# apache/datafusion-comet

Measured on NVIDIA H100. Metric: rows/sec on TPC-H Q1 filter+agg, higher is better.
Workload: dtype i128

## Files before the change

### datafusion-comet_b200/csrc/agg.cpp

```cpp
#include "exec_internal.h"
#include "../../include/comet_b200.h"

#include "aot_kernels.h"
#include "ranges.h"

#include <algorithm>
#include <mutex>

namespace cb200 {

static std::mutex g_profile_mu;
static std::map<std::string, std::vector<int>> g_range_profile;

void reset_range_profiles() {
    std::lock_guard<std::mutex> lk(g_profile_mu);
    g_range_profile.clear();
}

namespace {

enum class Strategy { Undecided, Dense, Table, Stream };
enum Level { SAFE = 0, TYPE = 1, TIGHT = 2 };
constexpr int DENSE_MAX_GROUPS = 64;

// ... 3 lines not shown

using ValueMasks = uint64_t[CB_MAX_COLS * 2];

uint64_t identity_word(int kind) { return kind == W_MIN ? 0x7fffffffffffffffull : kind == W_MAX ? 0x8000000000000000ull : 0; }

std::vector<int> decode_gid(int g, const std::vector<int>& cards) {
    std::vector<int> code(cards.size());
    for (int k = (int)cards.size() - 1; k >= 0; k--) { code[(size_t)k] = g % cards[(size_t)k]; g /= cards[(size_t)k]; }
    return code;
}

int grid_for(const ExecContext* ctx, int n_tiles) { return std::max(1, std::min(ctx->num_sms, n_tiles)); }

struct Kernel {
    PipelineSpec spec;
    GeneratedKernel g;
    std::shared_ptr<CompiledModule> mod;
};

void launch_named(ExecContext* ctx, const Kernel& k, const char* name, dim3 grid, dim3 block, void** args) {
    cuda_check(cudaLaunchKernel((const void*)k.mod->kernel(name), grid, block, args, 0, ctx->stream), name);
    ctx->kernel_launches++;
}

struct DenseState {
    std::vector<int> cards;
    std::vector<bool> has_null;
    DeviceBufP totals, spill, partials;
    int groups = 0;

    void regroup(ExecContext* ctx, int n_words, const std::vector<int>& word_kinds, const std::vector<int>& new_cards) {
        int new_groups = 1;
// ... 7 lines not shown
            for (int k = (int)cards.size() - 1; k >= 0; k--) {
                int cd = code[(size_t)k];
                if (has_null[(size_t)k] && cd == cards[(size_t)k] - 1) cd = new_cards[(size_t)k] - 1;
                ng += cd * mul;
                mul *= new_cards[(size_t)k];
            }
            memcpy(&newt[(size_t)ng * n_words * 2], &oldt[(size_t)g * n_words * 2], (size_t)n_words * 16);
        }
        totals = host_to_device(newt.data(), newt.size() * 8, ctx, "regroup H2D");
        groups = new_groups;
    }

    void finalize(ExecContext* ctx, const Kernel& last, cb::FinParams fp, bool ungrouped, const std::vector<DType>& schema,
                  const std::vector<DictionaryP>& key_dicts, Batch& out) const {
        TraceSpan ts("agg.finalize");
        const GeneratedKernel& g = last.g;
        const int ng = groups;
        fp.totals = (cb::u64*)totals->ptr;
        fp.n_groups = ng;
        std::vector<size_t> off_v, off_n;
        size_t total_bytes = 0;
        auto take = [&](size_t n) { size_t o = total_bytes; total_bytes += (n + 15) / 16 * 16; return o; };
        for (size_t i = 0; i < g.out_cols.size(); i++) { off_v.push_back(take((size_t)ng * g.out_bytes[i])); off_n.push_back(take((size_t)ng)); }
        size_t off_present = take((size_t)ng);
        auto dbuf = std::make_shared<DeviceBuf>(total_bytes);
        for (size_t i = 0; i < g.out_cols.size(); i++) {
            fp.out[i] = (cb::u8*)dbuf->ptr + off_v[i];
            fp.outv[i] = (cb::u8*)dbuf->ptr + off_n[i];
        }
        fp.present = (cb::u8*)dbuf->ptr + off_present;
        void* args[] = {&fp};
// ... 74 lines not shown
        bool overshoot = false;
        for (int r = 0; r < GK; r++) {
            if (hf.w[CB_HFLAG_CTR + r] > R || hf.w[CB_HFLAG_CTR + r] < 0) overshoot = true;
            cnt[r] = std::min<int64_t>(std::max(hf.w[CB_HFLAG_CTR + r], 0), R);
            if (hf.w[CB_HFLAG_CTR + r] < 0) cnt[r] = R;
            total += cnt[r];
        }
        if (overshoot && hflags) {
            for (int r = 0; r < GK; r++) hf.w[CB_HFLAG_CTR + r] = (int)cnt[r];
            write_flags(ctx, hf);
        }
        return total;
    }
    static void init_totals(ExecContext* ctx, const Kernel& k, cb::u64* totals, int64_t first, int64_t n) {
        if (n <= 0) return;
        const int n_words = k.g.n_words;
        if (std::none_of(k.g.word_kinds.begin(), k.g.word_kinds.end(), identity_word)) {
            cuda_check(cudaMemsetAsync(totals + first * n_words * 2, 0, (size_t)n * n_words * 16, ctx->stream), "memset totals");
        } else {
            long long f = first, nn = n;
            void* a1[] = {&totals, &f, &nn};
            launch_named(ctx, k, "cb_hash_init", dim3((unsigned)((n + 255) / 256)), dim3(256), a1);
        }
    }
    void grow(ExecContext* ctx, const Kernel& k, const int64_t cnt[GK], int64_t nm, bool zero_fill) {
        cudaStream_t st = ctx->stream;
        const int n_words = k.g.n_words, key_words = k.g.key_words;
        if (nm + 2 >= INT32_MAX) throw ExecError(16, "", "more than 2^31 groups in one partition; lower spark.comet.b200.chunkRows");
        const int64_t Ro = max_groups / GK, Rn = nm / GK;
        auto ntot = std::make_shared<DeviceBuf>((size_t)(nm + 2) * n_words * 16);
        auto nkog = std::make_shared<DeviceBuf>((size_t)nm * 8 * key_words + 16);
        cb::u64* tp = (cb::u64*)ntot->ptr;
        if (zero_fill) init_totals(ctx, k, tp, 0, nm + 2);
        else if (!htotals) init_totals(ctx, k, tp, nm, 2);
        if (htotals) {
            if (std::any_of(cnt, cnt + GK, [](int64_t c) { return c > 0; })) ctx->agg_table_grows++;
            for (int r = 0; r < GK; r++) {
                if (cnt[r] <= 0) continue;
                cuda_check(cudaMemcpyAsync(tp + (size_t)r * Rn * n_words * 2, (cb::u64*)htotals->ptr + (size_t)r * Ro * n_words * 2, (size_t)cnt[r] * n_words * 16,
                                           cudaMemcpyDeviceToDevice, st), "copy totals");
                cuda_check(cudaMemcpyAsync((cb::u64*)nkog->ptr + (size_t)r * Rn * key_words, (cb::u64*)hkey_of_gid->ptr + (size_t)r * Ro * key_words,
                                           (size_t)cnt[r] * 8 * key_words, cudaMemcpyDeviceToDevice, st), "copy group keys");
            }
            cuda_check(cudaMemcpyAsync(tp + (size_t)nm * n_words * 2, (cb::u64*)htotals->ptr + (size_t)max_groups * n_words * 2, (size_t)2 * n_words * 16,
                                       cudaMemcpyDeviceToDevice, st), "copy reserved groups");
        }
        cuda_check(cudaStreamSynchronize(st), "table growth");
        htotals = ntot; hkey_of_gid = nkog; max_groups = nm;
    }

    void finalize(ExecContext* ctx, const Kernel& last, cb::FinParams fp, const std::vector<DictionaryP>& key_dicts, Batch& out) {
        TraceSpan ts("agg.finalize_hash");
        const GeneratedKernel& g = last.g;
        HashFlags hfl;
        int64_t cnt[GK];
        const int64_t ng = read_flags(ctx, hfl, cnt);
        const int* flags = hfl.w;
        const int64_t n_out = ng + ((flags[0] & CB_HF_SENTINEL) ? 1 : 0) + ((flags[0] & CB_HF_NULL_GROUP) ? 1 : 0);
        fp.totals = (cb::u64*)htotals->ptr;
        fp.hkeys = (const cb::u64*)hkey_of_gid->ptr;
        fp.sentinel_used = flags[0] & CB_HF_SENTINEL;
        fp.null_group_used = (flags[0] & CB_HF_NULL_GROUP) ? 1 : 0;
        fp.n_hash_groups = (int)ng;
        fp.max_groups = (int)max_groups;
        fp.gid_range = (int)(max_groups / GK);
        int64_t run = 0;
        for (int r = 0; r < GK; r++) { fp.gid_prefix[r] = (int)run; run += cnt[r]; }
        fp.gid_prefix[GK] = (int)run;
// ... 101 lines not shown
    std::vector<AggExpr> aggs;
    std::vector<std::vector<int>> state_cols;
    AggMode mode = AggMode::Partial;
    bool reads_rows = true;
    bool all_partial = true;
    std::vector<bool> is_state_col;
    bool ungrouped = false;
    bool emitted = false;
    std::vector<Batch> outq;
    size_t outq_pos = 0;
    std::vector<int> assume_bits;

    std::vector<bool> key_has_null;
    std::vector<bool> col_nullable;
    std::vector<DictionaryP> key_dicts;
    struct DevDict { StringDictDev d; std::vector<DeviceBufP> bufs; int host_known = 0; };
    std::vector<std::shared_ptr<DevDict>> dev_dicts;

    int n_words = 0, key_words = 1;
    std::vector<int> word_kinds, role_words;
    Kernel last;
    bool have_totals() const { return last.mod != nullptr; }

    Strategy strategy = Strategy::Undecided;
    DenseState dense;
    KeyTable table;
    IdRows rows;

    std::vector<int> observed_bits;
    int64_t rows_scanned = 0;
    std::string profile_key;
// ... 30 lines not shown
                c.children = to_slots(a.children, slot_of);
                if (a.filter) c.filter = to_slots({a.filter}, slot_of)[0];
            }
            s.aggs.push_back(c);
        }
        for (auto& sc : state_cols) {
            std::vector<int> v;
            for (int ci : sc) v.push_back(slot_of.at(ci));
            s.state_slots.push_back(v);
        }
        if (hash) {
            s.threads = ctx->hash_threads;
            s.tile = 2 * ctx->hash_threads;
            s.stream = st == Strategy::Stream;
        }
        GeneratedKernel probe = generate_pipeline(s);
        size_t acc = (!ungrouped && !hash) ? (size_t)std::max(n_groups, 1) * probe.n_words * s.threads * 8 : 0;
        while (acc + 2 * (size_t)probe.stage_bytes + 1024 > SMEM_BUDGET && s.threads > 32) {
            s.threads /= 2;
            acc /= 2;
        }
        if (acc + 2 * (size_t)probe.stage_bytes + 1024 > SMEM_BUDGET)
            throw Unsupported(hash ? "too many state / input columns to stage in shared memory for the hash aggregate kernel"
                                   : "too many groups x aggregates for the thread-private accumulators of the dense path");
        s.stages = (int)std::max<size_t>(2, std::min<size_t>(6, (SMEM_BUDGET - 1024 - acc) / (size_t)probe.stage_bytes));
        return s;
    }

    std::vector<PipelineSpec> build_specs() const override {
        bool hash = false;
        for (auto& k : keys) if (!k->type.is_string() && k->type.id != TypeId::Bool) hash = true;
        std::vector<PipelineSpec> out{make_spec(nullptr, hash ? Strategy::Table : Strategy::Dense, ungrouped ? 1 : 6)};
        if (hash && mode == AggMode::Partial && all_partial) out.push_back(make_spec(nullptr, Strategy::Stream, 6));
        return out;
    }

    Kernel compile(const PipelineSpec& spec) {
        Kernel k{spec, generate_pipeline(spec), nullptr};
        k.mod = jit_get(k.g, true);
        if (have_totals() && k.g.key_words != key_words) throw ExecError(15, "", "internal: group key packing changed between launches");
        if (have_totals() && (k.g.n_words != n_words || k.g.word_kinds != word_kinds || k.g.role_words != role_words)) widen(k);
        n_words = k.g.n_words;
        word_kinds = k.g.word_kinds;
        role_words = k.g.role_words;
        key_words = k.g.key_words;
        return k;
    }

    void widen(const Kernel& k) {
        GeneratedKernel from;
        from.n_words = n_words;
        from.word_kinds = word_kinds;
        from.role_words = role_words;
        const std::vector<int> map = widen_word_map(from, k.g);
        if (map.empty()) throw ExecError(15, "", "internal: accumulator layout changed between launches");
        const bool is_dense = strategy == Strategy::Dense;
        DeviceBufP& t = is_dense ? dense.totals : rows.htotals;
        const size_t n_rows = is_dense ? (size_t)dense.groups : (size_t)rows.max_groups + 2;
        auto nt = std::make_shared<DeviceBuf>(n_rows * (size_t)k.g.n_words * 16);
        for (int w = 0; w < k.g.n_words; w++)
            cuda_check(cudaMemcpy2DAsync((char*)nt->ptr + (size_t)w * 16, (size_t)k.g.n_words * 16, (const char*)t->ptr + (size_t)map[(size_t)w] * 16,
                                         (size_t)n_words * 16, 16, n_rows, cudaMemcpyDeviceToDevice, ctx->stream), "widen totals");
        cuda_check(cudaStreamSynchronize(ctx->stream), "widen totals");
        t = nt;
    }

    void clear_vmask() {
        if (!vmask) vmask = std::make_shared<DeviceBuf>(CB_MAX_COLS * 16);
        cuda_check(cudaMemsetAsync(vmask->ptr, 0, CB_MAX_COLS * 16, ctx->stream), "memset vmask");
    }
    void copy_vmask(ValueMasks& masks) {
        cuda_check(cudaMemcpyAsync(masks, vmask->ptr, sizeof(ValueMasks), cudaMemcpyDeviceToHost, ctx->stream), "read value masks"); ctx->d2h_bytes += (int64_t)(sizeof(ValueMasks));
    }
    static std::vector<int> mask_bits(const PipelineSpec& spec, const ValueMasks& masks) {
        std::vector<int> seen(spec.cols.size(), -1);
        for (size_t i = 0; i < spec.cols.size(); i++) {
// ... 5 lines not shown
    }
    void observe(const std::vector<int>& seen) {
        for (size_t i = 0; i < seen.size(); i++)
            if (seen[i] >= 0) observed_bits[(size_t)used_cols[i]] = std::max(observed_bits[(size_t)used_cols[i]], seen[i]);
    }

    int prepare_key(Batch& b, size_t k) {
        int ci = keys[k]->index;
        Column& c = b.cols[ci];
        if (c.type.id == TypeId::Bool) return 2;
        if (!c.type.is_string()) return -1;
        if (c.is_dict) {
            key_dicts[k] = c.dict;
            return (int)c.dict->values().size();
        }
        if (!dev_dicts[k]) {
            auto dd = std::make_shared<DevDict>();
            const int64_t cap = 1 << 16;
            const int max_codes = 4096;
            const int64_t bytes_cap = 1 << 20;
            auto alloc = [&](size_t n) { auto bfr = std::make_shared<DeviceBuf>(n); cuda_check(cudaMemsetAsync(bfr->ptr, 0, bfr->bytes, ctx->stream), "memset dict"); dd->bufs.push_back(bfr); return bfr->ptr; };
            dd->d.tags = (unsigned long long*)alloc((size_t)cap * 8);
            dd->d.slot_code = (int*)alloc((size_t)cap * 4);
            dd->d.capacity = cap;
            dd->d.n_codes = (int*)alloc(64);
            dd->d.bytes_used = (unsigned long long*)((char*)dd->d.n_codes + 16);
            dd->d.err = (int*)((char*)dd->d.n_codes + 32);
            dd->d.max_codes = max_codes;
            dd->d.code_off = (long long*)alloc((size_t)max_codes * 8);
            dd->d.code_len = (int*)alloc((size_t)max_codes * 4);
            dd->d.bytes = (unsigned char*)alloc((size_t)bytes_cap);
            dd->d.bytes_cap = bytes_cap;
            dev_dicts[k] = dd;
            key_dicts[k] = std::make_shared<Dictionary>();
        }
        DevDict& dd = *dev_dicts[k];
        if (!c.offsets || !c.chars) throw Unsupported("string key column without offsets/chars buffers");
        auto row_slot = std::make_shared<DeviceBuf>((size_t)b.n_rows * 4);
        auto codes = std::make_shared<DeviceBuf>((size_t)b.n_rows * 4);
        launch_dict_encode(dd.d, (const int*)c.offsets->ptr, (const unsigned char*)c.chars->ptr, c.validity ? (const unsigned char*)c.validity->ptr : nullptr,
                           b.n_rows, (int*)row_slot->ptr, (int*)codes->ptr, ctx->stream);
        ctx->kernel_launches += 2;
        int hdr[12];
        cuda_check(cudaMemcpyAsync(hdr, dd.d.n_codes, sizeof(hdr), cudaMemcpyDeviceToHost, ctx->stream), "dict header");
        cuda_check(cudaStreamSynchronize(ctx->stream), "dict encode");
        int n_codes = hdr[0], derr = hdr[8];
        if (derr & CB_DICT_FULL) throw Unsupported("plain Utf8 group key with more distinct values than the device dictionary holds (dictionary-encode the column)");
        if (derr & CB_DICT_COLLISION) throw ExecError(14, "", "64-bit hash collision between distinct group key strings");
        if (n_codes > dd.host_known) {
            std::vector<long long> off((size_t)n_codes);
            std::vector<int> len((size_t)n_codes);
            cuda_check(cudaMemcpy(off.data(), dd.d.code_off, (size_t)n_codes * 8, cudaMemcpyDeviceToHost), "dict offsets");
            cuda_check(cudaMemcpy(len.data(), dd.d.code_len, (size_t)n_codes * 4, cudaMemcpyDeviceToHost), "dict lengths");
            for (int i = dd.host_known; i < n_codes; i++) {
                std::string s((size_t)len[(size_t)i], '\0');
                if (len[(size_t)i]) cuda_check(cudaMemcpy(&s[0], dd.d.bytes + off[(size_t)i], (size_t)len[(size_t)i], cudaMemcpyDeviceToHost), "dict bytes");
                key_dicts[k]->append(s);
            }
            dd.host_known = n_codes;
        }
        c.data = codes;
        c.phys = Phys::I32;
        c.is_dict = true;
        c.dict = key_dicts[k];
        return n_codes;
    }

    void consume(Batch& b) {
        for (int ci : used_cols) if (b.cols[(size_t)ci].validity) col_nullable[(size_t)ci] = true;
        std::vector<int> nc(keys.size());
        std::vector<bool> hn(keys.size());
        for (size_t k = 0; k < keys.size(); k++) {
// ... 22 lines not shown
        else if (strategy == Strategy::Table) consume_table(b);
        else consume_stream(b);
    }

    void consume_dense(Batch& b, const std::vector<int>& nc, int n_groups) {
        if (have_totals() && nc != dense.cards) {
            if (n_words == 0) throw ExecError(15, "", "internal: regroup before layout");
            dense.regroup(ctx, n_words, word_kinds, nc);
        }
        dense.cards = nc;
        dense.has_null = key_has_null;
        const int64_t SAMPLE = 1 << 20;
        bool have_obs = false;
        for (int ci : used_cols) if (child->schema[(size_t)ci].is_decimal() && observed_bits[(size_t)ci] >= 0) have_obs = true;
        if (reads_rows && !have_obs && b.n_rows > 2 * SAMPLE) {
            profile_key = pipeline_signature(make_spec(&b, Strategy::Dense, n_groups, SAFE));
            std::lock_guard<std::mutex> lk(g_profile_mu);
            auto it = g_range_profile.find(profile_key);
            if (it != g_range_profile.end() && it->second.size() == observed_bits.size()) {
                observed_bits = it->second;
                for (int ci : used_cols) if (child->schema[(size_t)ci].is_decimal() && observed_bits[(size_t)ci] >= 0) have_obs = true;
            }
        }
        if (!reads_rows) {
            run_range(b, 0, b.n_rows, n_groups, SAFE);
        } else if (!have_obs && b.n_rows > 2 * SAMPLE) {
            run_range(b, 0, SAMPLE, n_groups, TYPE);
            run_range(b, SAMPLE, b.n_rows, n_groups, TIGHT);
        } else {
            run_range(b, 0, b.n_rows, n_groups, have_obs ? TIGHT : TYPE);
// ... 13 lines not shown
            if (early.n_rows > 0) outq.push_back(std::move(early));
        }
        last = Kernel();
        dense = DenseState();
        n_words = 0; word_kinds.clear(); role_words.clear(); rows_scanned = 0;
    }

    void run_range(Batch& b, int64_t row0, int64_t row1, int n_groups, Level lv) {
        TraceSpan tsr("agg.run_range");
        while (true) {
            Kernel k;
            {
                TraceSpan ts("agg.codegen+jit");
                k = compile(make_spec(&b, Strategy::Dense, n_groups, lv));
            }
            const int64_t max_rows = (int64_t)ctx->num_sms * k.g.threads * (1ll << CB_RPT_LOG2) / 1024 * 1024;
            int64_t r0 = row0;
            while (r0 < row1 && launch_one(b, r0, std::min(row1, r0 + max_rows), n_groups, k, lv)) r0 += max_rows;
            if (r0 >= row1) return;
            if (lv == SAFE) throw ExecError(15, "", "internal: value-mask validation failed without assumptions");
            lv = lv == TIGHT ? TYPE : SAFE;
            row0 = r0;
        }
    }

    bool launch_one(Batch& b, int64_t r0, int64_t r1, int n_groups, const Kernel& k, Level lv) {
        cudaStream_t st = ctx->stream;
        size_t tot_bytes = (size_t)n_groups * n_words * 16;
        if (!have_totals()) {
            dense.totals = std::make_shared<DeviceBuf>(tot_bytes);
            dense.groups = n_groups;
        }
        if (!dense.spill || dense.spill->bytes < tot_bytes) {
            dense.spill = std::make_shared<DeviceBuf>(tot_bytes);
            cuda_check(cudaMemsetAsync(dense.spill->ptr, 0, dense.spill->bytes, st), "memset spill");
        }
        clear_vmask();
        cb::PipeParams p;
        fill_inputs(p, b, k.g.tile, r0, r1);
        bind_str_masks(p, k.spec, b);
        int grid = grid_for(ctx, p.n_tiles);
        size_t part_bytes = (size_t)grid * tot_bytes;
        if (!dense.partials || dense.partials->bytes < part_bytes) dense.partials = std::make_shared<DeviceBuf>(part_bytes);
        p.n_groups = n_groups;
        for (size_t i = 0; i < dense.cards.size() && i < CB_MAX_KEYS; i++) p.key_card[i] = dense.cards[i];
        p.partials = (cb::u8*)dense.partials->ptr;
        p.spill = (cb::u64*)dense.spill->ptr;
        p.vmask = (cb::u64*)vmask->ptr;
        launch(k.mod->kernel(k.g.entry), dim3(grid), dim3(k.g.threads + 32), k.g.dyn_smem(n_groups), &p);
        ctx->pipeline_rows += r1 - r0;
        ValueMasks masks;
        copy_vmask(masks);
        const int errs = ctx->take_device_errors();
        const std::vector<int> seen = mask_bits(k.spec, masks);
        bool ok = true;
        for (size_t i = 0; i < seen.size(); i++)
            if (k.spec.cols[i].assume_bits > 0 && seen[i] > k.spec.cols[i].assume_bits) ok = false;
        observe(seen);
        if (!ok) {
            cuda_check(cudaMemsetAsync(dense.spill->ptr, 0, dense.spill->bytes, st), "memset spill");
            ctx->agg_range_reruns++;
            return false;
        }
        ctx->raise_device_errors(errs);
// ... 7 lines not shown
        fp.n_ctas = grid;
        fp.n_groups = n_groups;
        fp.first = have_totals() ? 0 : 1;
        fp.err = ctx->d_err;
        int total_words = n_groups * n_words;
        void* args[] = {&fp};
        cuda_check(cudaLaunchKernel((const void*)k.mod->kernel("cb_fold"), dim3((total_words + 127) / 128), dim3(128), args, 0, st), "fold launch");
        ctx->kernel_launches++;
        last = k;
        return true;
    }

    void launch_id_rows(Batch& b, int64_t r0, int64_t r1, const Kernel& k, bool with_table) {
        clear_vmask();
        cb::PipeParams p;
        fill_inputs(p, b, k.g.tile, r0, r1);
        bind_str_masks(p, k.spec, b);
        p.hkeys = with_table ? (cb::u64*)table.hkeys->ptr : nullptr;
        p.hkey_of_gid = (cb::u64*)rows.hkey_of_gid->ptr;
        p.htotals = (cb::u64*)rows.htotals->ptr;
        p.hmask = with_table ? (cb::u32)(table.hcap - 1) : 0;
        p.max_groups = (cb::i32)rows.max_groups;
        p.hflags = (cb::i32*)rows.hflags->ptr;
        p.vmask = (cb::u64*)vmask->ptr;
        p.n_groups = 2;
        launch(k.mod->kernel(k.g.entry), dim3(grid_for(ctx, p.n_tiles)), dim3(k.g.threads + 32), k.g.dyn_smem(0), &p);
    }

    void consume_table(Batch& b) {
        const Kernel k = compile(make_spec(&b, Strategy::Table, 2, SAFE));
        {
            TraceSpan ts("hash.ensure_table");
            table.ensure(ctx, k, rows, b.n_rows, child->rows_hint(), rows_scanned, mode != AggMode::Partial || !all_partial);
        }
        launch_id_rows(b, 0, b.n_rows, k, true);
        ctx->pipeline_rows += b.n_rows;
        ValueMasks masks;
        int flags[8];
        copy_vmask(masks);
        cuda_check(cudaMemcpyAsync(flags, rows.hflags->ptr, sizeof(flags), cudaMemcpyDeviceToHost, ctx->stream), "read hash flags"); ctx->d2h_bytes += (int64_t)(sizeof(flags));
        ctx->check_device_errors();
// ... 182 lines not shown
```

### datafusion-comet_b200/csrc/codegen.cpp

```cpp
#include "codegen.h"
#include <mutex>
#include "device/cb_params.h"
#include "ranges.h"

#include <algorithm>
#include <climits>
#include <cstring>
#include <functional>
#include <memory>
#include <set>
#include <sstream>

namespace cb200 {

int phys_bytes(Phys p) {
    switch (p) {
    case Phys::Bitmap: return 0;
    case Phys::I8: return 1;
    case Phys::I16: return 2;
    case Phys::I32: case Phys::F32: case Phys::Dict32: return 4;
    case Phys::I64: case Phys::F64: return 8;
    case Phys::I128: return 16;
    }
    return 0;
// ... 677 lines not shown
std::string to_slot(const Val& v, const std::string& dst) {
    const DType& t = v.type;
    std::ostringstream o;
    if (t.is_decimal() && v.narrow) o << dst << "[0] = (cb::u64)" << v.v << "; " << dst << "[1] = (cb::u64)(" << v.v << " >> 63);";
    else if (t.is_decimal()) o << dst << "[0] = " << v.v << ".lo; " << dst << "[1] = (cb::u64)" << v.v << ".hi;";
    else if (t.id == TypeId::Float64) o << dst << "[0] = (cb::u64)__double_as_longlong(" << v.v << ");";
    else if (t.id == TypeId::Float32) o << dst << "[0] = (cb::u64)__float_as_uint(" << v.v << ");";
    else if (t.id == TypeId::Bool) o << dst << "[0] = " << v.v << " ? 1ull : 0ull;";
    else o << dst << "[0] = (cb::u64)(cb::i64)" << v.v << ";";
    return o.str();
}

}

namespace {
void sig_expr(std::ostringstream& o, const Expr& e) {
    uint64_t fb;
    memcpy(&fb, &e.lit_f64, 8);
    o << (int)e.kind << '|' << e.type.str() << '|' << e.index << '|' << e.lit_null << '|' << e.lit_i64 << '|' << fb << '|' << (uint64_t)e.lit_dec << ','
      << (uint64_t)(e.lit_dec >> 64) << '|' << e.lit_str << '|' << (int)e.eval_mode << '|' << e.fail_on_error << '|' << e.negated << '|' << e.wide_decimal << '|' << e.integral_div << e.check_divide_overflow << '|'
      << e.return_type.str() << '(';
    if (e.kind == ExprKind::StrPred) o << str_pred_key(e) << '|' << e.in_has_null << '|';
    for (auto& c : e.children) { sig_expr(o, *c); o << ','; }
    o << ')';
}
std::string spec_signature(const PipelineSpec& s) {
    std::ostringstream o;
    o << (int)s.sink << ';' << (int)s.mode << ';' << s.ungrouped << ';' << s.hash << (s.stream ? "s" : "") << (s.masked ? "m" : "") << ';' << s.tile << ';' << s.stages << ';' << s.threads << ';' << s.ltile << ";C";
    for (auto& c : s.cols) o << c.src_index << ':' << c.type.str() << ':' << (int)c.phys << ':' << c.has_validity << ':' << c.assume_bits << (c.layout_nullable && !c.has_validity ? "L" : "") << ',';
    o << ";P";
    for (auto& e : s.predicates) { sig_expr(o, *e); o << ';'; }
    o << ";O";
    for (auto& e : s.outputs) { sig_expr(o, *e); o << ';'; }
    o << ";K";
    for (size_t i = 0; i < s.keys.size(); i++) { sig_expr(o, *s.keys[i]); o << (i < s.key_nullable.size() && s.key_nullable[i]) << ';'; }
    o << ";A";
    for (auto& a : s.aggs) {
        o << (int)a.kind << ':' << (int)a.mode << ':' << a.datatype.str() << ':' << a.sum_datatype.str() << ':' << (int)a.eval_mode << '[';
        for (auto& c : a.children) { sig_expr(o, *c); o << ','; }
        o << "]F";
        if (a.filter) sig_expr(o, *a.filter);
        o << ';';
    }
    o << ";S";
    for (auto& v : s.state_slots) { for (int x : v) o << x << ','; o << ';'; }
    return o.str();
}
std::mutex g_memo_mu;
std::map<std::string, GeneratedKernel> g_memo;
GeneratedKernel generate_pipeline_uncached(const PipelineSpec& spec);
}

std::string pipeline_signature(const PipelineSpec& spec) { return spec_signature(spec); }

std::vector<int> widen_word_map(const GeneratedKernel& from, const GeneratedKernel& to) {
    if (from.role_words.size() != to.role_words.size()) return {};
    std::vector<int> map((size_t)to.n_words, -1);
    auto set = [&](int w, int o) {
        if (map[(size_t)w] >= 0 && map[(size_t)w] != o) return false;
        map[(size_t)w] = o;
        return true;
    };
    for (size_t r = 0; r < to.role_words.size(); r++) {
        const int w = to.role_words[r], o = from.role_words[r];
// ... 26 lines not shown
        for (auto& c : e->children) walk(c);
    };
    for (auto& e : spec.predicates) walk(e);
    for (auto& e : spec.outputs) walk(e);
    for (auto& e : spec.keys) walk(e);
    for (auto& a : spec.aggs)
        if (a.mode == AggMode::Partial) {
            for (auto& c : a.children) walk(c);
            walk(a.filter);
        }
    if (out.size() > CB_MAX_STR_PREDS)
        throw Unsupported("more than " + std::to_string(CB_MAX_STR_PREDS) + " distinct string predicates in one fused pipeline");
    return out;
}

GeneratedKernel generate_pipeline(const PipelineSpec& spec) {
    const std::string sig = spec_signature(spec);
    {
        std::lock_guard<std::mutex> lk(g_memo_mu);
        auto it = g_memo.find(sig);
        if (it != g_memo.end()) return it->second;
    }
    GeneratedKernel g = generate_pipeline_uncached(spec);
    std::lock_guard<std::mutex> lk(g_memo_mu);
    if (g_memo.size() > 4096) g_memo.clear();
    g_memo[sig] = g;
    return g;
}

namespace {
GeneratedKernel generate_pipeline_uncached(const PipelineSpec& spec) {
    GeneratedKernel g;
    g.threads = spec.threads;
    g.tile = spec.tile;
    g.stages = spec.stages;
    g.stage_bytes = stage_bytes_of(spec);
    if (spec.cols.empty()) throw Unsupported("pipeline without input columns");
    if (spec.cols.size() > 24) throw Unsupported("more than 24 staged input columns");

    Emitter em(spec);
    if (spec.sink == SinkKind::Agg && spec.hash) em.base_guard = "in_range";
    std::string keep = "true";
    for (auto& p : spec.predicates) {
// ... 525 lines not shown
```

### datafusion-comet_b200/csrc/codegen.h

```cpp
#pragma once
#include "plan.h"

#include <map>
#include <string>
#include <vector>

namespace cb200 {

enum class Phys { Bitmap, I8, I16, I32, I64, F32, F64, I128, Dict32 };
int phys_bytes(Phys p);

struct SourceCol {
    int src_index;
    DType type;
    Phys phys;
    bool has_validity;
    int assume_bits = 0;
    bool layout_nullable = false;
};

#define CB_RPT_LOG2 14

enum class SinkKind { Select, Agg, Count };

// ... 30 lines not shown
    int stage_bytes = 0;
    int n_words = 0;
    std::vector<int> word_kinds;
    std::vector<int> role_words;
    std::vector<OutCol> out_cols;
    std::vector<int> out_bytes;
    int threads = 256, tile = 512, stages = 3;
    bool hash = false;
    bool ungrouped = false;
    int n_key_cols = 0;
    int key_words = 1;
    size_t dyn_smem(int n_groups) const;
};

GeneratedKernel generate_pipeline(const PipelineSpec& spec);

std::vector<int> widen_word_map(const GeneratedKernel& from, const GeneratedKernel& to);

std::vector<ExprP> str_preds_of(const PipelineSpec& spec);
std::string str_pred_key(const Expr& e);
std::string pipeline_signature(const PipelineSpec& spec);

}
```

### datafusion-comet_b200/csrc/exec.cpp

```cpp
#include "exec_internal.h"

#include <cstdlib>
#include <ctime>
#include <mutex>

namespace cb200 {

enum { ERR_I128_OVERFLOW = 0, ERR_ANSI_OVERFLOW = 1, ERR_ORDER_DEPENDENT = 2, ERR_DIVIDE_BY_ZERO = 3, ERR_ARROW_DIVIDE_BY_ZERO = 4, ERR_DICT_CODE = 5,
       ERR_WIDE_MINMAX = 6 };

bool trace_on() {
    static int on = -1;
    if (on < 0) { const char* e = getenv("CB200_TRACE"); on = (e && *e && *e != '0') ? 1 : 0; }
    return on == 1;
}
double now_ms() {
    struct timespec ts;
    clock_gettime(CLOCK_MONOTONIC, &ts);
    return ts.tv_sec * 1e3 + ts.tv_nsec * 1e-6;
}
TraceSpan::TraceSpan(const char* n) : name(n), t0(trace_on() ? now_ms() : 0) {}
TraceSpan::~TraceSpan() {
    if (trace_on()) { static const double tz = now_ms(); const double t1 = now_ms(); fprintf(stderr, "[cb200 trace] %-28s %8.3f ms   (ends at +%.3f ms)\n", name, t1 - t0, t1 - tz); }
}
// ... 222 lines not shown
    }
    throw Unsupported("Arrow format '" + s + "' is outside the GPU hot path");
}

struct SchemaOnlySource : ExecNode {
    bool next(Batch&) override { return false; }
};

struct StreamSource : ExecNode {
    ExecContext* ctx;
    ArrowArrayStream* stream;
    bool schema_checked = false, eof = false;
    std::vector<bool> col_is_dict;
    std::vector<int> dict_index_width;
    std::vector<DictionaryP> dicts;

    StreamSource(ExecContext* c, ArrowArrayStream* s, const std::vector<DType>& fields) : ctx(c), stream(s) { schema = fields; }
    ~StreamSource() override {
        if (stream && stream->release) stream->release(stream);
    }

    void check_schema() {
        ArrowSchema sc;
        memset(&sc, 0, sizeof(sc));
        if (stream->get_schema(stream, &sc) != 0) {
            const char* m = stream->get_last_error ? stream->get_last_error(stream) : nullptr;
            throw ExecError(3, "", std::string("Failed to import ArrowArrayStream schema: ") + (m ? m : "?"));
        }
        if (sc.n_children != (int64_t)schema.size()) {
            int64_t n = sc.n_children;
            if (sc.release) sc.release(&sc);
            throw PlanError("scan declares " + std::to_string(schema.size()) + " fields but the stream has " + std::to_string(n));
        }
        col_is_dict.assign(schema.size(), false);
// ... 10 lines not shown
                dict_index_width[i] = it.arrow_width();
                if (it.arrow_width() == 8) throw Unsupported("int64 dictionary indices");
                dicts[i] = std::make_shared<Dictionary>();
            } else {
                DType t = dtype_from_format(ch->format);
                bool ok = t == schema[i] || (t.is_decimal() && schema[i].is_decimal() && t.scale == schema[i].scale) ||
                          (t.id == TypeId::Timestamp && schema[i].id == TypeId::TimestampNtz) || (t.id == TypeId::TimestampNtz && schema[i].id == TypeId::Timestamp);
                if (!ok) throw PlanError("scan field " + std::to_string(i) + " is " + schema[i].str() + " but the stream column is " + t.str());
            }
        }
        if (sc.release) sc.release(&sc);
        schema_checked = true;
    }

    bool next(Batch& out) override {
        if (!schema_checked) check_schema();
        if (eof) return false;
        std::vector<ArrowArray> arrs;
        int64_t total = 0;
        while (total < ctx->chunk_rows) {
            ArrowArray a;
            memset(&a, 0, sizeof(a));
            if (stream->get_next(stream, &a) != 0) {
                const char* m = stream->get_last_error ? stream->get_last_error(stream) : nullptr;
                for (auto& x : arrs) if (x.release) x.release(&x);
                throw ExecError(3, "", std::string("ArrowArrayStream get_next failed: ") + (m ? m : "?"));
            }
            if (!a.release) { eof = true; break; }
            if (a.length > 0) { total += a.length; arrs.push_back(a); }
            else a.release(&a);
        }
        if (arrs.empty()) return false;
        try {
            upload(arrs, total, out);
        } catch (...) {
            for (auto& x : arrs) if (x.release) x.release(&x);
            throw;
        }
        cuda_check(cudaStreamSynchronize(ctx->stream), "H2D copies");
        for (auto& x : arrs) if (x.release) x.release(&x);
        return true;
    }

    std::vector<int32_t> unify_dict(size_t col, const ArrowArray* d) {
        Dictionary& g = *dicts[col];
        const int32_t* off = (const int32_t*)d->buffers[1] + d->offset;
        const char* chars = (const char*)d->buffers[2];
        std::vector<int32_t> remap((size_t)d->length);
        bool identity = true;
        for (int64_t k = 0; k < d->length; k++) {
            const int32_t code = g.intern(std::string(chars + off[k], (size_t)(off[k + 1] - off[k])));
            remap[(size_t)k] = code;
            if (code != k) identity = false;
        }
        if (identity) remap.clear();
// ... 70 lines not shown
                if (total_chars > INT32_MAX) throw Unsupported("more than 2 GiB of string data in one chunk");
                col.chars = std::make_shared<DeviceBuf>((size_t)total_chars + 16);
                std::vector<int32_t> offs((size_t)total + 1);
                int64_t row = 0;
                int32_t base = 0;
                for (auto& a : arrs) {
                    ArrowArray* ch = a.children[c];
                    const int32_t* off = (const int32_t*)ch->buffers[1] + ch->offset;
                    for (int64_t i = 0; i < ch->length; i++) offs[(size_t)(row + i)] = base + (off[i] - off[0]);
                    int32_t nchars = off[ch->length] - off[0];
                    if (nchars) cuda_check(h2d((char*)col.chars->ptr + base, (const char*)ch->buffers[2] + off[0], (size_t)nchars), "H2D chars");
                    base += nchars;
                    row += ch->length;
                }
                offs[(size_t)total] = base;
                col.offsets = host_to_device(offs.data(), offs.size() * 4, ctx, "H2D offsets");
                ctx->h2d_bytes += (int64_t)(offs.size() * 4);
                col.phys = Phys::I32;
            } else {
                col.phys = phys_of(schema[c]);
                int w = schema[c].arrow_width();
                if (w == 0) {
                    col.data = std::make_shared<DeviceBuf>((size_t)(total + 7) / 8 + 8);
                    cuda_check(cudaMemsetAsync(col.data->ptr, 0, col.data->bytes, st), "memset bool");
                    int64_t row = 0;
                    for (auto& a : arrs) {
                        ArrowArray* ch = a.children[c];
                        append_bits((uint32_t*)col.data->ptr, row, (const uint8_t*)ch->buffers[1], ch->offset, ch->length, temps);
                        row += ch->length;
                    }
                } else {
                    col.data = std::make_shared<DeviceBuf>((size_t)total * w);
// ... 4 lines not shown
                        row += ch->length;
                    }
                }
            }
            if (any_nulls) {
                int64_t row = 0, nulls = 0;
                for (auto& a : arrs) {
                    ArrowArray* ch = a.children[c];
                    bool has = ch->null_count != 0 && ch->buffers[0];
                    append_bits((uint32_t*)col.validity->ptr, row, has ? (const uint8_t*)ch->buffers[0] : nullptr, ch->offset, ch->length, temps);
                    nulls += has ? (ch->null_count < 0 ? 1 : ch->null_count) : 0;
                    row += ch->length;
                }
                col.null_count = nulls;
            }
            if (!temps.empty()) cuda_check(cudaStreamSynchronize(st), "temp buffers");
        }
    }

    void append_bits(uint32_t* dst, int64_t row, const uint8_t* src, int64_t src_off, int64_t n, std::vector<DeviceBufP>& temps) {
        if (n <= 0) return;
        if (src && (row & 7) == 0 && (src_off & 7) == 0 && ((n & 7) == 0)) {
            cuda_check(h2d((char*)dst + (row >> 3), src + (src_off >> 3), (size_t)(n >> 3)), "H2D bitmap");
            return;
        }
        const uint8_t* dsrc = nullptr;
        int64_t doff = 0;
        if (src) {
            int64_t b0 = src_off >> 3, b1 = (src_off + n + 7) >> 3;
            auto tmp = std::make_shared<DeviceBuf>((size_t)(b1 - b0) + 8);
            temps.push_back(tmp);
// ... 467 lines not shown
```

Before: 35.76 billion.

## Cut host-side overhead in agg codegen memo, dict readback, and batch upload

Several host-side changes land together. The kernel memo now returns shared pointers instead of copying GeneratedKernel structs, and the signature builder uses to_chars in place of ostringstream. The device string dictionary moves into one buffer that is read back in a few bulk copies instead of one cudaMemcpy per string. Batch upload no longer synchronizes the stream; it records an event and holds the Arrow arrays until the next batch, so H2D copies can overlap host work. The deferred release adds lifetime risk: temp bitmap buffers are now freed without the per-column sync, and the offsets vectors must stay alive until the copy completes.

```diff
diff --git a/datafusion-comet_b200/csrc/agg.cpp b/datafusion-comet_b200/csrc/agg.cpp
--- a/datafusion-comet_b200/csrc/agg.cpp
+++ b/datafusion-comet_b200/csrc/agg.cpp
@@ -41,8 +41,9 @@
 
 struct Kernel {
     PipelineSpec spec;
-    GeneratedKernel g;
+    std::shared_ptr<const GeneratedKernel> gen;
     std::shared_ptr<CompiledModule> mod;
+    const GeneratedKernel& g() const { return *gen; }
 };
 
 void launch_named(ExecContext* ctx, const Kernel& k, const char* name, dim3 grid, dim3 block, void** args) {
@@ -80,7 +81,7 @@
     void finalize(ExecContext* ctx, const Kernel& last, cb::FinParams fp, bool ungrouped, const std::vector<DType>& schema,
                   const std::vector<DictionaryP>& key_dicts, Batch& out) const {
         TraceSpan ts("agg.finalize");
-        const GeneratedKernel& g = last.g;
+        const GeneratedKernel& g = last.g();
         const int ng = groups;
         fp.totals = (cb::u64*)totals->ptr;
         fp.n_groups = ng;
@@ -185,8 +186,8 @@
     }
     static void init_totals(ExecContext* ctx, const Kernel& k, cb::u64* totals, int64_t first, int64_t n) {
         if (n <= 0) return;
-        const int n_words = k.g.n_words;
-        if (std::none_of(k.g.word_kinds.begin(), k.g.word_kinds.end(), identity_word)) {
+        const int n_words = k.g().n_words;
+        if (std::none_of(k.g().word_kinds.begin(), k.g().word_kinds.end(), identity_word)) {
             cuda_check(cudaMemsetAsync(totals + first * n_words * 2, 0, (size_t)n * n_words * 16, ctx->stream), "memset totals");
         } else {
             long long f = first, nn = n;
@@ -196,7 +197,7 @@
     }
     void grow(ExecContext* ctx, const Kernel& k, const int64_t cnt[GK], int64_t nm, bool zero_fill) {
         cudaStream_t st = ctx->stream;
-        const int n_words = k.g.n_words, key_words = k.g.key_words;
+        const int n_words = k.g().n_words, key_words = k.g().key_words;
         if (nm + 2 >= INT32_MAX) throw ExecError(16, "", "more than 2^31 groups in one partition; lower spark.comet.b200.chunkRows");
         const int64_t Ro = max_groups / GK, Rn = nm / GK;
         auto ntot = std::make_shared<DeviceBuf>((size_t)(nm + 2) * n_words * 16);
@@ -222,7 +223,7 @@
 
     void finalize(ExecContext* ctx, const Kernel& last, cb::FinParams fp, const std::vector<DictionaryP>& key_dicts, Batch& out) {
         TraceSpan ts("agg.finalize_hash");
-        const GeneratedKernel& g = last.g;
+        const GeneratedKernel& g = last.g();
         HashFlags hfl;
         int64_t cnt[GK];
         const int64_t ng = read_flags(ctx, hfl, cnt);
@@ -354,7 +355,16 @@
     std::vector<bool> key_has_null;
     std::vector<bool> col_nullable;
     std::vector<DictionaryP> key_dicts;
-    struct DevDict { StringDictDev d; std::vector<DeviceBufP> bufs; int host_known = 0; };
+    struct DevDict {
+        static constexpr int64_t CAP = 1 << 16, MAX_CODES = 4096, BYTES_CAP = 1 << 20;
+        static constexpr size_t HDR = 64, OFF_TAGS = 0, OFF_SLOTS = CAP * 8, OFF_HDR = OFF_SLOTS + CAP * 4, TOTAL = OFF_HDR + HDR + MAX_CODES * 12 + BYTES_CAP;
+        static constexpr size_t S_CODE_OFF = HDR, S_CODE_LEN = S_CODE_OFF + MAX_CODES * 8, S_BYTES = S_CODE_LEN + MAX_CODES * 4;
+        StringDictDev d;
+        DeviceBufP buf;
+        int host_known = 0;
+        int64_t bytes_known = 0;
+        std::vector<uint8_t> stage;
+    };
     std::vector<std::shared_ptr<DevDict>> dev_dicts;
 
     int n_words = 0, key_words = 1;
@@ -415,7 +425,8 @@
             s.tile = 2 * ctx->hash_threads;
             s.stream = st == Strategy::Stream;
         }
-        GeneratedKernel probe = generate_pipeline(s);
+        const std::shared_ptr<const GeneratedKernel> probe_p = generate_pipeline_shared(s);
+        const GeneratedKernel& probe = *probe_p;
         size_t acc = (!ungrouped && !hash) ? (size_t)std::max(n_groups, 1) * probe.n_words * s.threads * 8 : 0;
         while (acc + 2 * (size_t)probe.stage_bytes + 1024 > SMEM_BUDGET && s.threads > 32) {
             s.threads /= 2;
@@ -437,14 +448,14 @@
     }
 
     Kernel compile(const PipelineSpec& spec) {
-        Kernel k{spec, generate_pipeline(spec), nullptr};
-        k.mod = jit_get(k.g, true);
-        if (have_totals() && k.g.key_words != key_words) throw ExecError(15, "", "internal: group key packing changed between launches");
-        if (have_totals() && (k.g.n_words != n_words || k.g.word_kinds != word_kinds || k.g.role_words != role_words)) widen(k);
-        n_words = k.g.n_words;
-        word_kinds = k.g.word_kinds;
-        role_words = k.g.role_words;
-        key_words = k.g.key_words;
+        Kernel k{spec, generate_pipeline_shared(spec), nullptr};
+        k.mod = jit_get(k.g(), true);
+        if (have_totals() && k.g().key_words != key_words) throw ExecError(15, "", "internal: group key packing changed between launches");
+        if (have_totals() && (k.g().n_words != n_words || k.g().word_kinds != word_kinds || k.g().role_words != role_words)) widen(k);
+        n_words = k.g().n_words;
+        word_kinds = k.g().word_kinds;
+        role_words = k.g().role_words;
+        key_words = k.g().key_words;
         return k;
     }
 
@@ -453,14 +464,14 @@
         from.n_words = n_words;
         from.word_kinds = word_kinds;
         from.role_words = role_words;
-        const std::vector<int> map = widen_word_map(from, k.g);
+        const std::vector<int> map = widen_word_map(from, k.g());
         if (map.empty()) throw ExecError(15, "", "internal: accumulator layout changed between launches");
         const bool is_dense = strategy == Strategy::Dense;
         DeviceBufP& t = is_dense ? dense.totals : rows.htotals;
         const size_t n_rows = is_dense ? (size_t)dense.groups : (size_t)rows.max_groups + 2;
-        auto nt = std::make_shared<DeviceBuf>(n_rows * (size_t)k.g.n_words * 16);
-        for (int w = 0; w < k.g.n_words; w++)
-            cuda_check(cudaMemcpy2DAsync((char*)nt->ptr + (size_t)w * 16, (size_t)k.g.n_words * 16, (const char*)t->ptr + (size_t)map[(size_t)w] * 16,
+        auto nt = std::make_shared<DeviceBuf>(n_rows * (size_t)k.g().n_words * 16);
+        for (int w = 0; w < k.g().n_words; w++)
+            cuda_check(cudaMemcpy2DAsync((char*)nt->ptr + (size_t)w * 16, (size_t)k.g().n_words * 16, (const char*)t->ptr + (size_t)map[(size_t)w] * 16,
                                          (size_t)n_words * 16, 16, n_rows, cudaMemcpyDeviceToDevice, ctx->stream), "widen totals");
         cuda_check(cudaStreamSynchronize(ctx->stream), "widen totals");
         t = nt;
@@ -496,23 +507,25 @@
             key_dicts[k] = c.dict;
             return (int)c.dict->values().size();
         }
+        TraceSpan ts("agg.prepare_key");
+        using DD = DevDict;
         if (!dev_dicts[k]) {
             auto dd = std::make_shared<DevDict>();
-            const int64_t cap = 1 << 16;
-            const int max_codes = 4096;
-            const int64_t bytes_cap = 1 << 20;
-            auto alloc = [&](size_t n) { auto bfr = std::make_shared<DeviceBuf>(n); cuda_check(cudaMemsetAsync(bfr->ptr, 0, bfr->bytes, ctx->stream), "memset dict"); dd->bufs.push_back(bfr); return bfr->ptr; };
-            dd->d.tags = (unsigned long long*)alloc((size_t)cap * 8);
-            dd->d.slot_code = (int*)alloc((size_t)cap * 4);
-            dd->d.capacity = cap;
-            dd->d.n_codes = (int*)alloc(64);
-            dd->d.bytes_used = (unsigned long long*)((char*)dd->d.n_codes + 16);
-            dd->d.err = (int*)((char*)dd->d.n_codes + 32);
-            dd->d.max_codes = max_codes;
-            dd->d.code_off = (long long*)alloc((size_t)max_codes * 8);
-            dd->d.code_len = (int*)alloc((size_t)max_codes * 4);
-            dd->d.bytes = (unsigned char*)alloc((size_t)bytes_cap);
-            dd->d.bytes_cap = bytes_cap;
+            dd->buf = std::make_shared<DeviceBuf>(DD::TOTAL);
+            uint8_t* base = (uint8_t*)dd->buf->ptr;
+            cuda_check(cudaMemsetAsync(base, 0, DD::OFF_HDR + DD::HDR, ctx->stream), "memset dict");
+            uint8_t* h = base + DD::OFF_HDR;
+            dd->d.n_codes = (int*)h;
+            dd->d.bytes_used = (unsigned long long*)(h + 16);
+            dd->d.err = (int*)(h + 32);
+            dd->d.tags = (unsigned long long*)(base + DD::OFF_TAGS);
+            dd->d.slot_code = (int*)(base + DD::OFF_SLOTS);
+            dd->d.capacity = DD::CAP;
+            dd->d.max_codes = (int)DD::MAX_CODES;
+            dd->d.code_off = (long long*)(h + DD::S_CODE_OFF);
+            dd->d.code_len = (int*)(h + DD::S_CODE_LEN);
+            dd->d.bytes = h + DD::S_BYTES;
+            dd->d.bytes_cap = DD::BYTES_CAP;
             dev_dicts[k] = dd;
             key_dicts[k] = std::make_shared<Dictionary>();
         }
@@ -523,21 +536,39 @@
         launch_dict_encode(dd.d, (const int*)c.offsets->ptr, (const unsigned char*)c.chars->ptr, c.validity ? (const unsigned char*)c.validity->ptr : nullptr,
                            b.n_rows, (int*)row_slot->ptr, (int*)codes->ptr, ctx->stream);
         ctx->kernel_launches += 2;
+        const uint8_t* base = (const uint8_t*)dd.buf->ptr + DD::OFF_HDR;
+        const int64_t bytes_bound = std::min<int64_t>(DD::BYTES_CAP, dd.bytes_known + (int64_t)c.chars->bytes);
+        const bool whole = (int64_t)DD::S_BYTES + bytes_bound <= (int64_t)256 << 10;
+        const size_t first = whole ? DD::S_BYTES + (size_t)bytes_bound : DD::HDR;
+        dd.stage.resize(std::max(dd.stage.size(), first));
+        cuda_check(cudaMemcpyAsync(dd.stage.data(), base, first, cudaMemcpyDeviceToHost, ctx->stream), "dict header");
+        cuda_check(cudaStreamSynchronize(ctx->stream), "dict encode");
         int hdr[12];
-        cuda_check(cudaMemcpyAsync(hdr, dd.d.n_codes, sizeof(hdr), cudaMemcpyDeviceToHost, ctx->stream), "dict header");
-        cuda_check(cudaStreamSynchronize(ctx->stream), "dict encode");
+        memcpy(hdr, dd.stage.data(), sizeof(hdr));
         int n_codes = hdr[0], derr = hdr[8];
         if (derr & CB_DICT_FULL) throw Unsupported("plain Utf8 group key with more distinct values than the device dictionary holds (dictionary-encode the column)");
         if (derr & CB_DICT_COLLISION) throw ExecError(14, "", "64-bit hash collision between distinct group key strings");
         if (n_codes > dd.host_known) {
-            std::vector<long long> off((size_t)n_codes);
-            std::vector<int> len((size_t)n_codes);
-            cuda_check(cudaMemcpy(off.data(), dd.d.code_off, (size_t)n_codes * 8, cudaMemcpyDeviceToHost), "dict offsets");
-            cuda_check(cudaMemcpy(len.data(), dd.d.code_len, (size_t)n_codes * 4, cudaMemcpyDeviceToHost), "dict lengths");
+            if (!whole) {
+                const size_t nn = (size_t)(n_codes - dd.host_known);
+                const uint64_t used = *(const uint64_t*)(dd.stage.data() + 16);
+                dd.stage.resize(std::max(dd.stage.size(), DD::S_BYTES + (size_t)used));
+                uint8_t* st = dd.stage.data();
+                cuda_check(cudaMemcpyAsync(st + DD::S_CODE_OFF + (size_t)dd.host_known * 8, base + DD::S_CODE_OFF + (size_t)dd.host_known * 8, nn * 8,
+                                           cudaMemcpyDeviceToHost, ctx->stream), "dict offsets");
+                cuda_check(cudaMemcpyAsync(st + DD::S_CODE_LEN + (size_t)dd.host_known * 4, base + DD::S_CODE_LEN + (size_t)dd.host_known * 4, nn * 4,
+                                           cudaMemcpyDeviceToHost, ctx->stream), "dict lengths");
+                if (used > (uint64_t)dd.bytes_known)
+                    cuda_check(cudaMemcpyAsync(st + DD::S_BYTES + dd.bytes_known, base + DD::S_BYTES + dd.bytes_known, (size_t)(used - dd.bytes_known),
+                                               cudaMemcpyDeviceToHost, ctx->stream), "dict bytes");
+                cuda_check(cudaStreamSynchronize(ctx->stream), "dict strings");
+            }
+            const long long* off = (const long long*)(dd.stage.data() + DD::S_CODE_OFF);
+            const int* len = (const int*)(dd.stage.data() + DD::S_CODE_LEN);
+            const char* bytes = (const char*)dd.stage.data() + DD::S_BYTES;
             for (int i = dd.host_known; i < n_codes; i++) {
-                std::string s((size_t)len[(size_t)i], '\0');
-                if (len[(size_t)i]) cuda_check(cudaMemcpy(&s[0], dd.d.bytes + off[(size_t)i], (size_t)len[(size_t)i], cudaMemcpyDeviceToHost), "dict bytes");
-                key_dicts[k]->append(s);
+                key_dicts[k]->append(std::string(bytes + off[i], (size_t)len[i]));
+                dd.bytes_known = std::max<int64_t>(dd.bytes_known, off[i] + len[i]);
             }
             dd.host_known = n_codes;
         }
@@ -590,6 +621,7 @@
         bool have_obs = false;
         for (int ci : used_cols) if (child->schema[(size_t)ci].is_decimal() && observed_bits[(size_t)ci] >= 0) have_obs = true;
         if (reads_rows && !have_obs && b.n_rows > 2 * SAMPLE) {
+            TraceSpan tsp("agg.range_profile");
             profile_key = pipeline_signature(make_spec(&b, Strategy::Dense, n_groups, SAFE));
             std::lock_guard<std::mutex> lk(g_profile_mu);
             auto it = g_range_profile.find(profile_key);
@@ -633,7 +665,7 @@
                 TraceSpan ts("agg.codegen+jit");
                 k = compile(make_spec(&b, Strategy::Dense, n_groups, lv));
             }
-            const int64_t max_rows = (int64_t)ctx->num_sms * k.g.threads * (1ll << CB_RPT_LOG2) / 1024 * 1024;
+            const int64_t max_rows = (int64_t)ctx->num_sms * k.g().threads * (1ll << CB_RPT_LOG2) / 1024 * 1024;
             int64_t r0 = row0;
             while (r0 < row1 && launch_one(b, r0, std::min(row1, r0 + max_rows), n_groups, k, lv)) r0 += max_rows;
             if (r0 >= row1) return;
@@ -644,6 +676,7 @@
     }
 
     bool launch_one(Batch& b, int64_t r0, int64_t r1, int n_groups, const Kernel& k, Level lv) {
+        TraceSpan ts("agg.launch_one");
         cudaStream_t st = ctx->stream;
         size_t tot_bytes = (size_t)n_groups * n_words * 16;
         if (!have_totals()) {
@@ -656,7 +689,7 @@
         }
         clear_vmask();
         cb::PipeParams p;
-        fill_inputs(p, b, k.g.tile, r0, r1);
+        fill_inputs(p, b, k.g().tile, r0, r1);
         bind_str_masks(p, k.spec, b);
         int grid = grid_for(ctx, p.n_tiles);
         size_t part_bytes = (size_t)grid * tot_bytes;
@@ -666,7 +699,7 @@
         p.partials = (cb::u8*)dense.partials->ptr;
         p.spill = (cb::u64*)dense.spill->ptr;
         p.vmask = (cb::u64*)vmask->ptr;
-        launch(k.mod->kernel(k.g.entry), dim3(grid), dim3(k.g.threads + 32), k.g.dyn_smem(n_groups), &p);
+        launch(k.mod->kernel(k.g().entry), dim3(grid), dim3(k.g().threads + 32), k.g().dyn_smem(n_groups), &p);
         ctx->pipeline_rows += r1 - r0;
         ValueMasks masks;
         copy_vmask(masks);
@@ -704,7 +737,7 @@
     void launch_id_rows(Batch& b, int64_t r0, int64_t r1, const Kernel& k, bool with_table) {
         clear_vmask();
         cb::PipeParams p;
-        fill_inputs(p, b, k.g.tile, r0, r1);
+        fill_inputs(p, b, k.g().tile, r0, r1);
         bind_str_masks(p, k.spec, b);
         p.hkeys = with_table ? (cb::u64*)table.hkeys->ptr : nullptr;
         p.hkey_of_gid = (cb::u64*)rows.hkey_of_gid->ptr;
@@ -714,7 +747,7 @@
         p.hflags = (cb::i32*)rows.hflags->ptr;
         p.vmask = (cb::u64*)vmask->ptr;
         p.n_groups = 2;
-        launch(k.mod->kernel(k.g.entry), dim3(grid_for(ctx, p.n_tiles)), dim3(k.g.threads + 32), k.g.dyn_smem(0), &p);
+        launch(k.mod->kernel(k.g().entry), dim3(grid_for(ctx, p.n_tiles)), dim3(k.g().threads + 32), k.g().dyn_smem(0), &p);
     }
 
     void consume_table(Batch& b) {
diff --git a/datafusion-comet_b200/csrc/codegen.cpp b/datafusion-comet_b200/csrc/codegen.cpp
--- a/datafusion-comet_b200/csrc/codegen.cpp
+++ b/datafusion-comet_b200/csrc/codegen.cpp
@@ -4,6 +4,7 @@
 #include "ranges.h"
 
 #include <algorithm>
+#include <charconv>
 #include <climits>
 #include <cstring>
 #include <functional>
@@ -715,7 +716,22 @@
 }
 
 namespace {
-void sig_expr(std::ostringstream& o, const Expr& e) {
+struct SigOut {
+    std::string s;
+    SigOut() { s.reserve(4096); }
+    SigOut& operator<<(char c) { s += c; return *this; }
+    SigOut& operator<<(bool b) { s += b ? '1' : '0'; return *this; }
+    SigOut& operator<<(const char* x) { s += x; return *this; }
+    SigOut& operator<<(const std::string& x) { s += x; return *this; }
+    template <class T, class = std::enable_if_t<std::is_integral<T>::value>>
+    SigOut& operator<<(T v) {
+        char buf[24];
+        const auto r = std::to_chars(buf, buf + sizeof(buf), v);
+        s.append(buf, r.ptr);
+        return *this;
+    }
+};
+void sig_expr(SigOut& o, const Expr& e) {
     uint64_t fb;
     memcpy(&fb, &e.lit_f64, 8);
     o << (int)e.kind << '|' << e.type.str() << '|' << e.index << '|' << e.lit_null << '|' << e.lit_i64 << '|' << fb << '|' << (uint64_t)e.lit_dec << ','
@@ -726,7 +742,7 @@
     o << ')';
 }
 std::string spec_signature(const PipelineSpec& s) {
-    std::ostringstream o;
+    SigOut o;
     o << (int)s.sink << ';' << (int)s.mode << ';' << s.ungrouped << ';' << s.hash << (s.stream ? "s" : "") << (s.masked ? "m" : "") << ';' << s.tile << ';' << s.stages << ';' << s.threads << ';' << s.ltile << ";C";
     for (auto& c : s.cols) o << c.src_index << ':' << c.type.str() << ':' << (int)c.phys << ':' << c.has_validity << ':' << c.assume_bits << (c.layout_nullable && !c.has_validity ? "L" : "") << ',';
     o << ";P";
@@ -745,10 +761,10 @@
     }
     o << ";S";
     for (auto& v : s.state_slots) { for (int x : v) o << x << ','; o << ';'; }
-    return o.str();
+    return std::move(o.s);
 }
 std::mutex g_memo_mu;
-std::map<std::string, GeneratedKernel> g_memo;
+std::map<std::string, std::shared_ptr<const GeneratedKernel>> g_memo;
 GeneratedKernel generate_pipeline_uncached(const PipelineSpec& spec);
 }
 
@@ -805,19 +821,21 @@
     return out;
 }
 
-GeneratedKernel generate_pipeline(const PipelineSpec& spec) {
+std::shared_ptr<const GeneratedKernel> generate_pipeline_shared(const PipelineSpec& spec) {
     const std::string sig = spec_signature(spec);
     {
         std::lock_guard<std::mutex> lk(g_memo_mu);
         auto it = g_memo.find(sig);
         if (it != g_memo.end()) return it->second;
     }
-    GeneratedKernel g = generate_pipeline_uncached(spec);
+    auto g = std::make_shared<const GeneratedKernel>(generate_pipeline_uncached(spec));
     std::lock_guard<std::mutex> lk(g_memo_mu);
     if (g_memo.size() > 4096) g_memo.clear();
     g_memo[sig] = g;
     return g;
 }
+
+GeneratedKernel generate_pipeline(const PipelineSpec& spec) { return *generate_pipeline_shared(spec); }
 
 namespace {
 GeneratedKernel generate_pipeline_uncached(const PipelineSpec& spec) {
diff --git a/datafusion-comet_b200/csrc/codegen.h b/datafusion-comet_b200/csrc/codegen.h
--- a/datafusion-comet_b200/csrc/codegen.h
+++ b/datafusion-comet_b200/csrc/codegen.h
@@ -68,6 +68,7 @@
 };
 
 GeneratedKernel generate_pipeline(const PipelineSpec& spec);
+std::shared_ptr<const GeneratedKernel> generate_pipeline_shared(const PipelineSpec& spec);
 
 std::vector<int> widen_word_map(const GeneratedKernel& from, const GeneratedKernel& to);
 
diff --git a/datafusion-comet_b200/csrc/exec.cpp b/datafusion-comet_b200/csrc/exec.cpp
--- a/datafusion-comet_b200/csrc/exec.cpp
+++ b/datafusion-comet_b200/csrc/exec.cpp
@@ -260,10 +260,22 @@
     std::vector<bool> col_is_dict;
     std::vector<int> dict_index_width;
     std::vector<DictionaryP> dicts;
+    std::vector<ArrowArray> held;
+    std::vector<std::vector<int32_t>> held_offsets;
+    cudaEvent_t uploaded = nullptr;
 
     StreamSource(ExecContext* c, ArrowArrayStream* s, const std::vector<DType>& fields) : ctx(c), stream(s) { schema = fields; }
     ~StreamSource() override {
+        release_held();
+        if (uploaded) cudaEventDestroy(uploaded);
         if (stream && stream->release) stream->release(stream);
+    }
+    void release_held() {
+        if (held.empty() && held_offsets.empty()) return;
+        cudaEventSynchronize(uploaded);
+        for (auto& x : held) if (x.release) x.release(&x);
+        held.clear();
+        held_offsets.clear();
     }
 
     void check_schema() {
@@ -304,7 +316,9 @@
     }
 
     bool next(Batch& out) override {
+        TraceSpan ts("source.next");
         if (!schema_checked) check_schema();
+        release_held();
         if (eof) return false;
         std::vector<ArrowArray> arrs;
         int64_t total = 0;
@@ -324,11 +338,14 @@
         try {
             upload(arrs, total, out);
         } catch (...) {
+            cudaStreamSynchronize(ctx->stream);
             for (auto& x : arrs) if (x.release) x.release(&x);
+            held_offsets.clear();
             throw;
         }
-        cuda_check(cudaStreamSynchronize(ctx->stream), "H2D copies");
-        for (auto& x : arrs) if (x.release) x.release(&x);
+        if (!uploaded) cuda_check(cudaEventCreateWithFlags(&uploaded, cudaEventDisableTiming), "cudaEventCreate");
+        cuda_check(cudaEventRecord(uploaded, ctx->stream), "event record");
+        held = std::move(arrs);
         return true;
     }
 
@@ -429,8 +446,10 @@
                     row += ch->length;
                 }
                 offs[(size_t)total] = base;
-                col.offsets = host_to_device(offs.data(), offs.size() * 4, ctx, "H2D offsets");
+                col.offsets = std::make_shared<DeviceBuf>(offs.size() * 4);
+                cuda_check(cudaMemcpyAsync(col.offsets->ptr, offs.data(), offs.size() * 4, cudaMemcpyHostToDevice, st), "H2D offsets");
                 ctx->h2d_bytes += (int64_t)(offs.size() * 4);
+                held_offsets.push_back(std::move(offs));
                 col.phys = Phys::I32;
             } else {
                 col.phys = phys_of(schema[c]);
@@ -465,7 +484,6 @@
                 }
                 col.null_count = nulls;
             }
-            if (!temps.empty()) cuda_check(cudaStreamSynchronize(st), "temp buffers");
         }
     }
 
```

After: 37.79 billion (median of 6 runs). 5.7% higher.
